# Fytex/Shafa-CD

Measured on AMD Instinct MI355X. Metric: GiB/s Shannon-Fano encode+decode, 64 MiB blocks, 1/2/4/8 GPUs; bit-exact, higher is better.
Workload: dtype u8

## Files before the change

### shafa-cd_amd/csrc/sf_decode.hip

```cpp
#include <type_traits>
#include "common.hpp"
#include "internal.hpp"

#include <atomic>
#include <mutex>
#include <thread>

#include <algorithm>

#include <stdlib.h>

#include "sfd_common.hpp"
#include "sfd_dp.hpp"
#include "sfd_generic.hpp"

namespace {

typedef __attribute__((address_space(3))) u32 lds_u32;
typedef __attribute__((address_space(3))) u16 lds_u16;
typedef __attribute__((address_space(3))) u8 lds_u8;
template <int LONG> constexpr u32 spec_emask() { return LONG == 2 ? 31u : 15u; }

constexpr int SC_PHW = 16;
constexpr int SC_M = 4;
// ... 470 lines not shown
{
    const u32 mask = (1u << KW) - 1u;
    auto long_len = [&](const u32 qq) -> u32 {
        const u32 win = __builtin_bitreverse32(sw.at(qq));
        const u32 l = (LONG == 1 ? long_code(lt, win) : long_code32(lt, win)) >> 8;
        return l ? l : 1u;
    };
    const u32 nlook = KW <= 10 ? 3u : 2u;
    while (q + nlook * KW <= qe && (int)(q + nlook * KW) <= qlimit) {
        const u32 w = sw.at(q);
        u32 sum = 0, e = 0;
        for (u32 i = 0; i < nlook; ++i) {
            e = tab[(w >> (sum & 31u)) & mask];
            sum += e;
        }
        q += sum & 31u;
        cnt += sum >> 5;
        if (LONG && __builtin_expect((e & 31u) == 0u, 0)) {
            const u32 l = long_len(q);
            if ((int)(q + l) > qlimit) { q = qe + spec_emask<LONG>(); return; }
            q += l;
            ++cnt;
        }
    }
    const lds_u8 *len0 = tab + (1u << KW);
    while (q < qe) {
        u32 l0 = len0[sw.at(q) & mask];
        if (LONG && __builtin_expect(l0 == 0u, 0)) l0 = long_len(q);
        if ((int)(q + l0) > qlimit) { q = qe + spec_emask<LONG>(); break; }
        q += l0;
        ++cnt;
    }
}

template <bool HAVE_OLD, int LONG>
__device__ __forceinline__ void sl_strip(const lds_u8 *tab, const u16 *lt, const u32 KW, const u32 qrow, const int qlimit, const u32 ent0,
                                         u32 (&ent)[2], u32 (&cnt)[2], u32 &exit_)
{
    u32 q = qrow + ent0;
    SlWin sw;
    sw.init();
#pragma unroll
    for (int k = 0; k < 2; ++k) {
        const u32 r = q - (qrow + 256u * k);
        if (HAVE_OLD && k > 0 && r == ent[k]) return;
        ent[k] = r;
        u32 c = 0;
        sl_walk<LONG>(tab, lt, KW, q, qrow + 256u * (k + 1), qlimit, c, sw);
        cnt[k] = c;
    }
    exit_ = (q - (qrow + 512u)) & spec_emask<LONG>();
}

template <int LONG>
__device__ __forceinline__ u32 sl_region(u8 *smem, const DecBlk &blk, const u32 tile0, const u32 e0_forced, u8 *__restrict__ chunk_entry,
                                         u16 *__restrict__ chunk_cnt, u32 *__restrict__ tile_cnt, u8 *__restrict__ tile_guess,
                                         u8 *__restrict__ tile_exit, const u32 tab_bytes)
{
    const u64 start = (u64)tile0 * DTILE;
    const u64 left = blk.in_n > start ? blk.in_n - start : 0;
    const size_t gt0 = (size_t)blk.tile_base + tile0;
    const u32 ntl = blk.n_tiles - tile0 < (u32)SC_WTILES ? blk.n_tiles - tile0 : (u32)SC_WTILES;
    u32 *data = (u32 *)smem;
    const u32 tab_off = SL_LDS_DATA;
    u8 *ex = smem + SL_LDS_DATA + tab_bytes;
    const u32 tid = threadIdx.x, lane = tid & 63, wv = tid >> 6;
    const u32 KW = blk.KW;
    const u16 *lt = (const u16 *)(smem + SL_LDS_DATA + tab_bytes + SL_MISC);
    {
        const long long base = (long long)start - 4 * SL_SW;
        constexpr u32 UNITS = (u32)(SL_STRIPS * SL_SW / 4 + 1), NIT = (UNITS + DEC_THREADS - 1) / DEC_THREADS;
        uint4 v[NIT];
#pragma unroll
        for (u32 it = 0; it < NIT; ++it) {
            const u32 i = tid + it * DEC_THREADS;
            const long long off = base + (long long)i * 16;
            v[it] = make_uint4(0, 0, 0, 0);
            if (i < UNITS && off >= 0 && (u64)off + 16 <= blk.in_n) v[it] = gload<uint4>(blk.in + off);
        }
#pragma unroll
        for (u32 it = 0; it < NIT; ++it) {
            const u32 i = tid + it * DEC_THREADS;
            if (i >= UNITS) break;
            const long long off = base + (long long)i * 16;
            u32 w[4] = {v[it].x, v[it].y, v[it].z, v[it].w};
            if (off >= 0 && (u64)off < blk.in_n && (u64)off + 16 > blk.in_n) {
                const int nv = (int)(blk.in_n - (u64)off);
#pragma unroll
                for (int q = 0; q < 16; ++q)
                    if (q < nv) w[q >> 2] |= (u32)gload<u8>(blk.in + off + q) << (8 * (q & 3));
            }
            const u32 f = 4 * i, at = f + f / SL_SW;
            const u32 w0 = rev_bytes(w[0]);
            if (f % SL_SW == 0 && f > 0) data[at - 1] = w0;
            if (i < UNITS - 1) {
                data[at] = w0;
                data[at + 1] = rev_bytes(w[1]);
                data[at + 2] = rev_bytes(w[2]);
                data[at + 3] = rev_bytes(w[3]);
            }
        }
    }
    __syncthreads();
    const int limit = (int)(left * 8) - (int)(512u * tid);
    const u32 qrow = 8u * ((4u * SL_ROW) * (tid + 1));
    const int qlimit = (int)qrow + limit;
    const lds_u8 *tab = (const lds_u8 *)(size_t)tab_off;
    u32 ent[2] = {0, 0}, cnt[2] = {0, 0}, exit_ = 0;
    {
        u32 e0;
        if (tid == 0) e0 = e0_forced;
        else {
            const u32 qe = qrow;
            u32 q = qe - 256u, dummy = 0;
            SlWin sw;
            sw.init();
            sl_walk<LONG>(tab, lt, KW, q, qe, qlimit, dummy, sw);
            e0 = (q - qe) & spec_emask<LONG>();
        }
        sl_strip<false, LONG>(tab, lt, KW, qrow, qlimit, e0, ent, cnt, exit_);
    }
    ex[tid] = (u8)exit_;
    __syncthreads();
    bool bad = false;
    u32 *const wsum = (u32 *)(ex + DEC_THREADS), *const flags = wsum + 4;
    u32 turn = 0;
    for (int round = 0; round < 4; ++round) {
        bad = tid > 0 && ent[0] != (u32)ex[tid - 1];
        if (!wg_any(bad, flags, turn)) break;
        if (bad) sl_strip<true, LONG>(tab, lt, KW, qrow, qlimit, (u32)ex[tid - 1], ent, cnt, exit_);
        __syncthreads();
        ex[tid] = (u8)exit_;
        __syncthreads();
        bad = tid > 0 && ent[0] != (u32)ex[tid - 1];
    }
    if (wg_any(bad, flags, turn)) {
        if (tid == 0) __hip_atomic_store(blk.run_dp, 1u, __ATOMIC_RELAXED, __HIP_MEMORY_SCOPE_AGENT);
    }
    const u32 my_tile = tid / 128u;
    const u32 wtot = dpp_scan_add(cnt[0] + cnt[1]);
    if (lane == 63) wsum[wv] = wtot;
    __syncthreads();
    if (my_tile < ntl) {
        const size_t c0 = gt0 * DEC_THREADS + (size_t)tid * 2;
        gstore<u16>(chunk_entry + c0, (u16)((ent[0] & 0xFFu) | (ent[1] << 8)));
        gstore<u32>(chunk_cnt + c0, cnt[0] | (cnt[1] << 16));
        const u32 in_tile = tid & 127u;
        if (in_tile == 0) {
            tile_cnt[gt0 + my_tile] = wsum[2 * my_tile] + wsum[2 * my_tile + 1];
            tile_guess[gt0 + my_tile] = (u8)ent[0];
        }
        if (in_tile == 127u) tile_exit[gt0 + my_tile] = (u8)exit_;
    }
    const u32 unit_exit = ex[ntl * 128u - 1u];
    __syncthreads();
    return unit_exit;
}

constexpr u32 SF_CHUNKS = 8;

constexpr u32 SF_LINKS = 2 * DEC_THREADS;
template <int LONG>
__device__ __forceinline__ void sf_links(u8 *smem, const DecBlk &blk, const u32 t_begin, const u32 t_end, u8 *__restrict__ chunk_entry,
                                         u16 *__restrict__ chunk_cnt, u32 *__restrict__ tile_cnt, u8 *__restrict__ tile_guess,
                                         const u8 *__restrict__ tile_exit, const u32 tab_bytes, const u32 long_bytes)
{
    const u32 tid = threadIdx.x, KW = blk.KW, mask = (1u << KW) - 1u;
    const u16 *lt = (const u16 *)(smem + tab_bytes + 48);
    const u8 *len0 = smem + (1u << KW);
    const u64 end_bit = blk.in_n * 8;
    u32 turn = 0;
    u32 xs[SF_LINKS / DEC_THREADS];
    bool any_bad = false;
#pragma unroll
    for (u32 i = 0; i < SF_LINKS / DEC_THREADS; ++i) {
        const u32 t = t_begin + tid + i * DEC_THREADS;
        xs[i] = 0xFFFFFFFFu;
        if (t < t_end) {
            const size_t gt = (size_t)blk.tile_base + t;
            const u32 x = tile_exit[gt - 1];
            if (tile_guess[gt] != x) { xs[i] = x; any_bad = true; }
        }
    }
    if (!wg_any(any_bad, (u32 *)(smem + tab_bytes), turn)) return;
    __syncthreads();
    fill_lds16((void *)smem, (const void *)blk.cnt3, 2u << KW);
    if (LONG) {
        const u16 *src = LONG == 1 ? blk.longtab : blk.long32;
        if (src) fill_lds16((void *)lt, src, long_bytes);
        else if (tid == 0) *(u16 *)lt = 0;
    }
    bool failed = false;
    volatile u32 *const gave_up = (volatile u32 *)(smem + tab_bytes + 32);
    if (tid == 0) *gave_up = 0;
    __syncthreads();
#pragma unroll 1
    for (u32 i = 0; i < SF_LINKS / DEC_THREADS; ++i) {
        if (*gave_up) break;
        const u32 x = xs[i];
        if (x == 0xFFFFFFFFu) continue;
        const u32 t = t_begin + tid + i * DEC_THREADS;
        const size_t gt = (size_t)blk.tile_base + t;
        const u64 tile_bit0 = (u64)t * DTILE * 8;
        if (x >= spec_emask<LONG>() || tile_bit0 + (u64)(SF_CHUNKS + 1) * CH_BITS + 64 > end_bit) { failed = true; *gave_up = 1; continue; }
        u32 q = x, wi = 0xFFFFFFFFu, lo = 0, hi = 0;
        auto window = [&](const u32 qq) -> u32 {
            const u32 i = qq >> 5;
            if (i != wi) {
                const u8 *p = blk.in + (u64)t * DTILE + 4u * i;
                lo = rev_bytes(gload<u32>(p));
                hi = rev_bytes(gload<u32>(p + 4));
                wi = i;
            }
            return __builtin_amdgcn_alignbit(hi, lo, qq);
        };
        int delta = 0;
        bool merged = false;
        const size_t c0 = gt * DEC_THREADS;
        for (u32 c = 0; c < SF_CHUNKS; ++c) {
            const u32 qe = CH_BITS * (c + 1);
            u32 cnt = 0;
            while (q < qe) {
                const u32 w = window(q);
                u32 l = len0[w & mask];
                if (LONG && l == 0u) {
                    const u32 win = __builtin_bitreverse32(w);
                    l = (LONG == 1 ? long_code(lt, win) : long_code32(lt, win)) >> 8;
                    if (!l) l = 1u;
                }
                q += l;
                ++cnt;
            }
            delta += (int)cnt - (int)chunk_cnt[c0 + c];
            chunk_cnt[c0 + c] = (u16)cnt;
            const u32 e = q - qe;
            if (e == (u32)chunk_entry[c0 + c + 1]) { merged = true; break; }
            chunk_entry[c0 + c + 1] = (u8)e;
        }
        if (!merged) { failed = true; *gave_up = 1; continue; }
        chunk_entry[c0] = (u8)x;
        tile_guess[gt] = (u8)x;
        tile_cnt[gt] = (u32)((int)tile_cnt[gt] + delta);
    }
    if (wg_any(failed, (u32 *)(smem + tab_bytes), turn) && tid == 0)
        __hip_atomic_store(blk.run_dp, 1u, __ATOMIC_RELAXED, __HIP_MEMORY_SCOPE_AGENT);
}

template <int LONG>
__global__ __launch_bounds__(DEC_THREADS) void sfd_ends(const DecBlk *__restrict__ blks, u8 *__restrict__ chunk_entry,
                                                        u16 *__restrict__ chunk_cnt, u32 *__restrict__ tile_cnt,
                                                        u8 *__restrict__ tile_guess, u8 *__restrict__ tile_exit, u32 tab_bytes, u32 long_bytes)
{
    extern __shared__ __attribute__((aligned(16))) u8 smem[];
    const DecBlk blk = blks[blockIdx.y];
    if (!blk.n_tiles || !blk.run_dp || __hip_atomic_load(blk.run_dp, __ATOMIC_RELAXED, __HIP_MEMORY_SCOPE_AGENT) != 0) return;
    if (lds_addr(smem) != 0) __builtin_trap();
    const u32 units = (blk.n_tiles + SC_WTILES - 1) / SC_WTILES;
    u32 first_end = units - 1;
    if (units >= 2 && blk.in_n - (u64)(units - 2) * SC_WTILES * DTILE < (u64)64 * SC_SB + 4) first_end = units - 2;
    if (blockIdx.x > 0) {
        const u32 t_end = first_end * SC_WTILES, t_begin = 1u + (blockIdx.x - 1u) * SF_LINKS;
        if (t_begin < t_end)
            sf_links<LONG>(smem, blk, t_begin, t_end, chunk_entry, chunk_cnt, tile_cnt, tile_guess, tile_exit, tab_bytes, long_bytes);
        return;
    }
    fill_lds16((void *)(smem + SL_LDS_DATA), (const void *)blk.cnt3, 2u << blk.KW);
    if (LONG) {
        u16 *lt = (u16 *)(smem + SL_LDS_DATA + tab_bytes + SL_MISC);
        const u16 *src = LONG == 1 ? blk.longtab : blk.long32;
        if (src) fill_lds16((void *)lt, src, long_bytes);
        else if (threadIdx.x == 0) *lt = 0;
    }
    __syncthreads();
    u32 e0 = first_end ? (u32)tile_exit[(size_t)blk.tile_base + first_end * SC_WTILES - 1] : 0u;
    for (u32 u = first_end; u < units; ++u)
        e0 = sl_region<LONG>(smem, blk, u * SC_WTILES, e0, chunk_entry, chunk_cnt, tile_cnt, tile_guess, tile_exit, tab_bytes);
}

constexpr int ws_row(bool esc) { return CH_BYTES / 4 + (esc ? 3 : 2); }
constexpr int ws_rows_bytes(bool esc)
{
    return 16 + (DEC_THREADS * ws_row(esc) + (esc ? 0 : DEC_THREADS / 16)) * 4;
}
constexpr int WS_MISC = 32;
typedef unsigned int u32x3_t __attribute__((ext_vector_type(3)));
constexpr u32 WS_NST = 4, WS_DROP = 0x7FFFFFF0u;
constexpr int WS_RSRC_FLAGS = 0x00020000, WS_AUX_NT = 2;

__device__ __forceinline__ void ws_walk1(const u32 tab_off, const u32 mask2, const u32 xa, u32 q2, const u32 q2end, u32 want,
                                         const bool by_pos)
{
    auto window2 = [&]() -> u32 {
        const lds_u32 *pa = (const lds_u32 *)(size_t)((q2 >> 3) & ~3u);
        return __builtin_amdgcn_alignbit(pa[1], pa[0], q2);
    };
    auto look = [&](const u32 w) -> u32 { return *(const lds_u16 *)(size_t)(tab_off + (w & mask2)); };
    auto image_or = [](const u32 at, const u32 v) {
        __hip_atomic_fetch_or((lds_u32 *)(size_t)at, v, __ATOMIC_RELAXED, __HIP_MEMORY_SCOPE_WORKGROUP);
    };
    if (by_pos) {
        constexpr u32 N = 3, F = 4, WPG = F * N / 4;
        const u32 s = (0u - xa) & 3u;
        u32 ptr = ((xa + 3u) & ~3u) - 4u;
        u32 L = 0, Lp = 0, Ep = 0;
        auto group = [&](auto first_group) -> bool {
            constexpr bool FIRST = decltype(first_group)::value;
            u32 x0 = 0, x1 = 0, ub = 0;
#pragma unroll
            for (u32 f = 0; f < F; ++f) {
                if (!((int)q2 < (int)q2end)) {
                    if (f == 0) {
                        if (!FIRST) {
                            image_or(ptr + 4u * (WPG - 1u), Ep);
                            image_or(ptr + 4u * WPG, __builtin_amdgcn_alignbyte(0u, Lp, s));
                        }
                    } else {
                        const u32 at = ptr + 4u * (f * N >> 2);
                        image_or(at, __builtin_amdgcn_alignbyte(L, Lp, s));
                        image_or(at + 4u, __builtin_amdgcn_alignbyte(0u, L, s));
                    }
                    return false;
                }
                if (f == 0 && !FIRST) {
                    *(lds_u32 *)(size_t)(ptr + 4u * (WPG - 1u)) = Ep;
                    ptr += 4u * WPG;
                }
                u32 w;
                if ((f & 1u) == 0) {
                    const lds_u32 *pa = (const lds_u32 *)(size_t)((q2 >> 3) & ~3u);
                    const u32 w0 = pa[0], w1 = pa[1], w2 = pa[2];
                    w = x0 = __builtin_amdgcn_alignbit(w1, w0, q2);
                    x1 = __builtin_amdgcn_alignbit(w2, w1, q2);
                } else
                    w = __builtin_amdgcn_alignbit(x1, x0, ub);
                u32 ua = 0;
#pragma unroll
                for (u32 i = 0; i < N; ++i) {
                    const u32 k = f * N + i, b = k & 3u;
                    const u32 e = look(w >> ua);
                    ua += e >> 8;
                    L = __builtin_amdgcn_perm(e, L, b == 0 ? 0x0C0C0C04u : b == 1 ? 0x0C0C0400u : b == 2 ? 0x0C040100u : 0x04020100u);
                    if (b == 3u) {
                        const u32 E = __builtin_amdgcn_alignbyte(L, Lp, s), at = ptr + 4u * (k >> 2);
                        Lp = L;
                        if (FIRST && k == 3u) image_or(at, E);
                        else if (k == F * N - 1u) Ep = E;
                        else *(lds_u32 *)(size_t)at = E;
                    }
                }
                q2 += ua;
                ub = ua;
            }
            return true;
        };
        if (group(std::true_type{}))
            while (group(std::false_type{})) {}
        return;
    }
    u32 wp = xa & ~3u, nb = 8u * (xa & 3u), acc = 0;
    for (; want; --want) {
        const u32 e = look(window2());
        q2 += e >> 8;
        acc |= (e & 0xFFu) << nb;
        nb += 8u;
        if (nb == 32u) {
            image_or(wp, acc);
            wp += 4u;
            acc = nb = 0;
        }
    }
    if (nb) image_or(wp, acc);
}

template <int LONG, bool ESC, bool ONE = false>
__global__ __launch_bounds__(DEC_THREADS) void sfd_wstage(const DecBlk *__restrict__ blks, const u8 *__restrict__ chunk_entry,
                                                          const u16 *__restrict__ chunk_cnt, const u64 *__restrict__ tile_off,
                                                          u32 tpw, u32 tab_bytes, u32 cap, u32 long_bytes)
{
    extern __shared__ __attribute__((aligned(16))) u8 smem[];
    const DecBlk blk = blks[blockIdx.y];
    const u32 first_tile = blockIdx.x * tpw;
    if (first_tile >= blk.n_tiles) return;
    if (tile_off[(size_t)blk.tile_base + first_tile] >= blk.n_sym) return;
    const u32 LONGB = LONG ? long_bytes : 0u;
    u32 *rows = (u32 *)(smem + 16);
    constexpr u32 WS_ROW = (u32)ws_row(ESC), tab_off = (u32)ws_rows_bytes(ESC);
    const u16 *lt = (const u16 *)(smem + tab_off + tab_bytes);
    const u32 img_off = tab_off + tab_bytes + LONGB;
    u32 *wsum = (u32 *)(smem + img_off + cap);
    u32 *next = wsum + 4;
    const u32 tid = threadIdx.x, lane = tid & 63, wv = tid >> 6;
    const u32 K1 = blk.K1, K3 = sym3_window(K1);
    const u32 sh = 32 - K1;
    static_assert(!ONE || (LONG == 0 && !ESC), "the one-code walk has no escapes");
    constexpr bool one = ONE;
    fill_lds16(smem + tab_off, (const void *)blk.sym3, (one ? 2u : 4u) << K3);
    if (LONG) {
        const u16 *src = LONG == 1 ? blk.longtab : blk.long32;
        if (src) fill_lds16((void *)lt, src, LONGB);
        else if (tid == 0) *(u16 *)lt = 0;
    }
    for (u32 i = tid; i < cap / 16; i += DEC_THREADS) *(uint4 *)(smem + img_off + 16 * i) = make_uint4(0, 0, 0, 0);
    bool bad = false;
    if (lds_addr(smem) != 0) __builtin_trap();
    const u32 q2row = 8u * (16u + 4u * (WS_ROW * tid + (ESC ? 0u : tid >> 4))) - (one ? 1u : 2u);
    const u32 mask4 = ((1u << K3) - 1u) << (one ? 1 : 2);
    auto fetch16 = [&](const u64 off) -> uint4 {
        if (off + 16 <= blk.in_n) return gload_nt<uint4>(blk.in + off);
        u32 w[4] = {0, 0, 0, 0};
        if (off < blk.in_n) {
            const int nv = (int)(blk.in_n - off);
#pragma unroll
            for (int q = 0; q < 16; ++q)
                if (q < nv) w[q >> 2] |= (u32)gload<u8>(blk.in + off + q) << (8 * (q & 3));
        }
        return make_uint4(w[0], w[1], w[2], w[3]);
    };
    uint4 pf0, pf1;
    u32 pf2[ESC ? 3 : 2] = {};
    auto fetch_ahead = [&](const u64 off) {
        constexpr int NB = ESC ? 12 : 8;
        if (off + NB <= blk.in_n) {
            if constexpr (ESC) {
                const u32x3_t v = __builtin_nontemporal_load((const GLOBAL_AS u32x3_t *)(unsigned long long)(blk.in + off));
                pf2[0] = v.x; pf2[1] = v.y; pf2[2] = v.z;
            } else {
                const uint2 v = gload_nt<uint2>(blk.in + off);
                pf2[0] = v.x; pf2[1] = v.y;
            }
            return;
        }
        u32 w[3] = {0, 0, 0};
        if (off < blk.in_n) {
            const int nv = (int)(blk.in_n - off);
#pragma unroll
            for (int q = 0; q < NB; ++q)
                if (q < nv) w[q >> 2] |= (u32)gload<u8>(blk.in + off + q) << (8 * (q & 3));
        }
#pragma unroll
        for (int q = 0; q < NB / 4; ++q) pf2[q] = w[q];
    };
    u8 pf_entry = 0, pf_next = 0;
    u16 pf_cnt = 0;
    auto prefetch = [&](const u32 tile) {
        const u64 base = (u64)tile * DTILE;
        const size_t g = ((size_t)blk.tile_base + tile) * DEC_THREADS + tid;
        pf_entry = chunk_entry[g];
        pf_cnt = chunk_cnt[g];
        pf_next = (tile + 1 < blk.n_tiles || tid + 1 < (u32)DEC_THREADS) ? chunk_entry[g + 1] : (u8)0;
        pf0 = fetch16(base + 16ull * tid);
        pf1 = fetch16(base + 16ull * (tid + DEC_THREADS));
        if (tid == 0) fetch_ahead(base + DTILE);
    };
    auto put16 = [&](const u32 i, const uint4 v) {
        const u32 f = 4 * i, at = f + (WS_ROW - 8u) * (f >> 3) + (ESC ? 0u : f >> 7);
        const u32 w0 = rev_bytes(v.x), w1 = rev_bytes(v.y), w2 = rev_bytes(v.z);
        if ((f & 7u) == 0 && f > 0) {
            const u32 lk = at - (WS_ROW - 8u) - (!ESC && (f & 127u) == 0 ? 1u : 0u);
            rows[lk] = w0;
            rows[lk + 1] = w1;
            if (ESC) rows[lk + 2] = w2;
        }
        if (i < (u32)(DTILE / 16)) {
            rows[at] = w0;
            rows[at + 1] = w1;
            rows[at + 2] = w2;
            rows[at + 3] = rev_bytes(v.w);
        }
    };
    auto store_bytes = [&](u8 *ga, const uint4 v, const u32 lo, const u32 hi) {
        const u32 wds[4] = {v.x, v.y, v.z, v.w};
#pragma unroll
        for (u32 q = 0; q < 16; ++q)
            if (q >= lo && q < hi) gstore<u8>(ga + q, (u8)(wds[q >> 2] >> (8 * (q & 3))));
    };
    u32 carry_n = 0, carry_lo = 0;
    u8 *carry_g = nullptr;
    prefetch(first_tile);
    __builtin_amdgcn_s_waitcnt(0x0F70);
    for (u32 it = 0; it < tpw; ++it) {
        const u32 tile = first_tile + it;
        if (tile >= blk.n_tiles) break;
        const size_t gt = (size_t)blk.tile_base + tile;
        const u64 toff = tile_off[gt];
        if (toff >= blk.n_sym) break;
        lds_barrier();
        put16(tid, pf0);
        put16(tid + DEC_THREADS, pf1);
        if (tid == 0) put16(DTILE / 16, make_uint4(pf2[0], pf2[1], ESC ? pf2[ESC ? 2 : 0] : 0u, 0u));
        const u32 entry = pf_entry, cnt = pf_cnt, nent = pf_next;
        if (it + 1 < tpw && tile + 1 < blk.n_tiles) prefetch(tile + 1);
        const u32 incl = wave_incl_scan_add<u32>(cnt);
        if (lane == 63) wsum[wv] = incl;
        lds_barrier();
        u32 pre = incl - cnt, total = 0;
        for (u32 w = 0; w < 4; ++w) { if (w < wv) pre += wsum[w]; total += wsum[w]; }
        const u64 room = blk.n_sym - toff;
        const u32 tot_c = (u32)__builtin_amdgcn_readfirstlane((int)(room < (u64)total ? (u32)room : total));
        u32 want = pre >= tot_c ? 0u : (tot_c - pre < cnt ? tot_c - pre : cnt);
        u32 q2 = q2row + entry;
        const bool by_pos = want == cnt && tile + 1 < blk.n_tiles && nent != spec_emask<LONG>();
        const u32 q2end = q2row + 256u + nent;
        u32 done = 0;
        do {
            u8 *gout = blk.out + toff + done;
            const u32 mis = (u32)((uintptr_t)gout & 15u);
            if (carry_g && (carry_n != mis || carry_g != gout - mis)) {
                if (tid == 0) {
                    uint4 *ip = (uint4 *)(smem + img_off);
                    store_bytes(carry_g, *ip, carry_lo, carry_n);
                    ip[0] = make_uint4(0, 0, 0, 0);
                    ip[1] = make_uint4(0, 0, 0, 0);
                }
                carry_n = 0;
                carry_g = nullptr;
                lds_barrier();
            }
            const u32 capw = cap - 32;
            u32 nxt = tot_c;
            if (mis + (tot_c - done) > capw) {
                if (tid == 0) *next = tot_c;
                lds_barrier();
                if (want && pre >= done && mis + (pre - done) + want > capw) atomicMin(next, pre);
                lds_barrier();
                nxt = (u32)__builtin_amdgcn_readfirstlane((int)*next);
                lds_barrier();
            }
            const bool mine = want && pre >= done && pre + want <= nxt;
            if constexpr (ONE) {
                if (mine) ws_walk1(tab_off, mask4, img_off + mis + (pre - done), q2, q2end, want, by_pos);
            } else if (mine) {
                const u32 x = mis + (pre - done);
                u32 wp = img_off + (x & ~3u), nbx = x << 30, acc = 0;
                auto emit = [&](const u32 e) {
                    const u32 sh = nbx >> 27, syms = e & 0xFFFFFFu;
                    acc |= syms << sh;
                    if (__builtin_add_overflow(nbx, e & 0xC0000000u, &nbx)) {
                        __hip_atomic_fetch_or((lds_u32 *)(size_t)wp, acc, __ATOMIC_RELAXED, __HIP_MEMORY_SCOPE_WORKGROUP);
                        wp += 4u;
                        acc = syms >> (32u - sh);
                    }
                };
                auto window4 = [&]() -> u32 {
                    const lds_u32 *pa = (const lds_u32 *)(size_t)((q2 >> 3) & ~3u);
                    return __builtin_amdgcn_alignbit(pa[1], pa[0], q2);
                };
                auto step = [&](const bool tail) {
                    u32 e = *(const lds_u32 *)(size_t)(tab_off + (window4() & mask4));
                    if (ESC && __builtin_expect((e >> 30) == 0, 0)) {
                        const u32 q = q2 + 2u;
                        const lds_u32 *pb = (const lds_u32 *)(size_t)((q >> 3) & ~3u);
                        const u32 win = __builtin_bitreverse32(__builtin_amdgcn_alignbit(pb[1], pb[0], q));
                        u32 e1 = LONG == 1 ? long_code(lt, win) : LONG == 2 ? long_code32(lt, win)
                                           : (u32)gload<u16>(blk.lut13 + (win >> sh));
                        if (e1 == 0) { bad = true; e1 = 1u << 8; }
                        e = (e1 & 0xFFu) | ((e1 >> 8) << 24) | (1u << 30);
                    }
                    u32 n = e >> 30, syms = e & 0xFFFFFFu;
                    if (tail) {
                        n = n < want ? n : want;
                        syms &= (1u << (8 * n)) - 1u;
                    }
                    emit(syms | n << 30);
                    q2 += (e >> 24) & 63u;
                    want -= n;
                };
                auto multi = [&](auto nlook) {
                    constexpr u32 N = decltype(nlook)::value;
                    if (by_pos) {
                        while ((int)q2 < (int)q2end) {
                            const u32 w4 = window4();
                            u32 ua = 0, e = 0;
#pragma unroll
                            for (u32 i = 0; i < N; ++i) {
                                e = *(const lds_u32 *)(size_t)(tab_off + ((w4 >> (ua & 31u)) & mask4));
                                emit(e);
                                ua += e >> 24;
                            }
                            q2 += ua & 63u;
                            if (ESC && __builtin_expect((e >> 30) == 0, 0)) step(false);
                        }
                        want = 0;
                    }
                    while (want >= 3 * N) {
                        const u32 w4 = window4();
                        u32 ua = 0, e = 0;
#pragma unroll
                        for (u32 i = 0; i < N; ++i) {
                            e = *(const lds_u32 *)(size_t)(tab_off + ((w4 >> (ua & 31u)) & mask4));
                            emit(e);
                            ua += e >> 24;
                        }
                        q2 += ua & 63u;
                        want -= ua >> 6;
                        if (ESC && __builtin_expect((e >> 30) == 0, 0)) step(false);
                    }
                };
                if (K3 <= 10) multi(std::integral_constant<u32, 3>{});
                else if (K3 <= 15) multi(std::integral_constant<u32, 2>{});
                while (want) step(true);
                if (nbx) __hip_atomic_fetch_or((lds_u32 *)(size_t)wp, acc, __ATOMIC_RELAXED, __HIP_MEMORY_SCOPE_WORKGROUP);
            }
            lds_barrier();
            const u32 end = mis + (nxt - done);
            const u32 lo0 = (carry_n == mis && carry_n) ? carry_lo : mis;
            const u32 nfull = end >> 4;
            u8 *const g0 = gout - mis;
            if constexpr (LONG == 2) {
                for (u32 u = tid; u < nfull; u += DEC_THREADS) {
                    uint4 *ip = (uint4 *)(smem + img_off + 16 * u);
                    const uint4 v = *ip;
                    *ip = make_uint4(0, 0, 0, 0);
                    if (u == 0 && lo0) store_bytes(g0, v, lo0, 16u);
                    else gstore_nt<uint4>(g0 + 16 * u, v);
                }
            } else {
                const __amdgpu_buffer_rsrc_t win = __builtin_amdgcn_make_buffer_rsrc(g0, 0, (int)(16u * nfull), WS_RSRC_FLAGS);
                u32 ub = tid;
                do {
#pragma unroll
                    for (u32 s = 0; s < WS_NST; ++s) {
                        const u32 u = ub + s * DEC_THREADS;
                        u32x4_t x = {0u, 0u, 0u, 0u};
                        u32 off = WS_DROP;
                        if (u < nfull) {
                            uint4 *ip = (uint4 *)(smem + img_off + 16 * u);
                            const uint4 v = *ip;
                            *ip = make_uint4(0, 0, 0, 0);
                            if (s == 0 && u == 0 && lo0) store_bytes(g0, v, lo0, 16u);
                            else {
                                x.x = v.x; x.y = v.y; x.z = v.z; x.w = v.w;
                                off = 16u * u;
                            }
                        }
                        __builtin_amdgcn_raw_buffer_store_b128(x, win, (int)off, 0, WS_AUX_NT);
                    }
                    ub += WS_NST * DEC_THREADS;
                } while (__builtin_amdgcn_readfirstlane((int)(ub - tid)) < (int)nfull);
            }
            if (tid == 0 && nfull) {
                uint4 *ip = (uint4 *)(smem + img_off);
                const uint4 a = ip[nfull], b = ip[nfull + 1];
                ip[nfull] = make_uint4(0, 0, 0, 0);
                ip[nfull + 1] = make_uint4(0, 0, 0, 0);
                ip[0] = a;
                ip[1] = b;
            }
            carry_lo = nfull ? 0u : lo0;
            carry_n = end & 15u;
            carry_g = g0 + 16 * nfull;
            done = nxt;
            if (done < tot_c) lds_barrier();
        } while (done < tot_c);
    }
    if (tid == 0 && carry_n) {
        const uint4 v = *(const uint4 *)(smem + img_off);
        store_bytes(carry_g, v, carry_lo, carry_n);
    }
    if (bad) set_error(blk.err, SHAFA_FILE_UNRECOGNIZABLE);
}

__global__ __launch_bounds__(DEC_THREADS) void sfd_offsets(const DecBlk *__restrict__ blks,
                                                           const u32 *__restrict__ tile_cnt, u64 *__restrict__ tile_off)
{
    __shared__ u64 wtot[4];
    __shared__ u64 carry;
    const DecBlk blk = blks[blockIdx.x];
    const u32 tid = threadIdx.x, lane = tid & 63, wv = tid >> 6;
    if (tid == 0) carry = 0;
    __syncthreads();
    constexpr u32 OFF_EPT = 16;
    for (u32 r0 = 0; r0 < blk.n_tiles; r0 += DEC_THREADS * OFF_EPT) {
        const u32 t0 = r0 + tid * OFF_EPT;
        u32 x[OFF_EPT];
#pragma unroll
        for (u32 j = 0; j < OFF_EPT; ++j) x[j] = t0 + j < blk.n_tiles ? tile_cnt[blk.tile_base + t0 + j] : 0u;
        u64 mine = 0;
#pragma unroll
        for (u32 j = 0; j < OFF_EPT; ++j) mine += x[j];
        const u64 incl = wave_incl_scan_add<u64>(mine);
        if (lane == 63) wtot[wv] = incl;
        __syncthreads();
        u64 base = carry + incl - mine;
        for (u32 w = 0; w < wv; ++w) base += wtot[w];
#pragma unroll
        for (u32 j = 0; j < OFF_EPT; ++j) {
            if (t0 + j < blk.n_tiles) tile_off[blk.tile_base + t0 + j] = base;
            base += x[j];
        }
        __syncthreads();
        if (tid == 0) carry += wtot[0] + wtot[1] + wtot[2] + wtot[3];
        __syncthreads();
    }
    if (tid == 0 && carry < blk.n_sym) set_error(blk.err, SHAFA_FILE_UNRECOGNIZABLE);
}

}

#include "sfd_host_tables.hpp"

template <class F> static void for_blocks_parallel(int nblocks, F fn)
{
    std::atomic<int> next{0};
    auto work = [&]() {
        for (;;) {
            const int b = next.fetch_add(1, std::memory_order_relaxed);
            if (b >= nblocks) break;
            fn(b);
        }
    };
    int helpers = nblocks / 16;
    const int hw = (int)std::thread::hardware_concurrency();
    if (helpers > 7) helpers = 7;
    if (hw > 0 && helpers > hw - 1) helpers = hw - 1;
    std::vector<std::thread> th;
    for (int i = 0; i < helpers; ++i) {
        try { th.emplace_back(work); } catch (...) { break; }
    }
    work();
    for (auto &t : th) t.join();
}

static int g_sfd_speculate = 1;
void sfdec_configure(int speculate) { g_sfd_speculate = speculate; }
static int g_sfd_path = 0;
void sfdec_configure_path(int path) { g_sfd_path = path; }

static bool spec_worthwhile(const shafa_code_table &t, const HostTab &h, bool force)
{
    if (!h.ok || !(h.complete || h.complete16 || h.complete32) || h.lmax > 32 || h.lmax < 2) return false;
    if (force) return true;
    const u64 key = spec_key(t.len, t.bits);
    static u64 ckey[1024];
    static signed char cval[1024];
    static std::mutex cmu;
    const u32 slot = (u32)(key >> 17) & 1023u;
    {
        std::lock_guard<std::mutex> lk(cmu);
        if (cval[slot] && ckey[slot] == key) return cval[slot] == 2;
    }
    u64 rs = key | 1ull;
    int fails = 0;
    for (int trial = 0; trial < SPEC_TRIALS && fails <= SPEC_MAX_FAILS; ++trial) {
        u64 w[SPEC_WORDS];
        for (u64 &x : w) x = spec_rand(rs);
        if (!spec_trial(w, h.lenlut.data(), h.K1)) ++fails;
    }
    const bool yes = fails <= SPEC_MAX_FAILS;
    std::lock_guard<std::mutex> lk(cmu);
    ckey[slot] = key;
    cval[slot] = yes ? 2 : 1;
    return yes;
}

struct SfdArrays {
    u8 *cfn, *tfn;
    u8 *tent, *cent;
    u16 *ccnt;
    u32 *tcnt;
    u64 *toff;
    u8 *tguess, *texit;
};

enum SfdForm { SFD_MID32, SFD_LONG_ALL, SFD_PACKED12, SFD_PACKED13, SFD_PACKED };

static u32 sfd_tpw(u32 most, u32 max_tiles, int nblocks)
{
    u32 tpw = most;
    while (tpw > 1 && (u64)ceil_div_u64(max_tiles, tpw) * nblocks < 2048) tpw >>= 1;
    return tpw;
}

static void sfd_launch_packed(hipStream_t st, const DecBlk *dblk, int nblocks, u32 max_tiles, SfdForm form, bool esc, bool spec,
                              u32 tabb, u32 long_used, bool all_spec, u32 ws_tab, u32 ws_cap, const SfdArrays &a, bool one = false)
{
    static decltype(&sfd_scan<0>) const scans[3] = {sfd_scan<2>, sfd_scan<1>, sfd_scan<0>};
    static decltype(&sfd_ends<0>) const ends[3] = {sfd_ends<2>, sfd_ends<1>, sfd_ends<0>};
    static decltype(&sfd_sync16<true, false>) const syncs[4] = {sfd_sync16<false, true>, sfd_sync16<true, false, 12>,
                                                                sfd_sync16<true, false, 13>, sfd_sync16<true, false>};
    const int f = form < SFD_PACKED12 ? form : 2;
    const dim3 grid_b((u32)nblocks), wg(DEC_THREADS);
    hipLaunchKernelGGL(sfd_tables, dim3((u32)nblocks, 8), wg, 0, st, dblk);
    if (spec) {
        const size_t lds_scan = (size_t)SC_LDS_ROWS + tabb + SC_MISC + long_used;
        const size_t lds_ends = (size_t)SL_LDS_DATA + tabb + SL_MISC + long_used;
        hipLaunchKernelGGL(scans[f], dim3((u32)ceil_div_u64(max_tiles, SC_TILES), (u32)nblocks), wg, lds_scan, st, dblk, a.cent, a.ccnt,
                           a.tcnt, a.tguess, a.texit, tabb, long_used);
        hipLaunchKernelGGL(ends[f], dim3(1u + (u32)ceil_div_u64(max_tiles, SF_LINKS), (u32)nblocks), wg, lds_ends, st, dblk, a.cent,
                           a.ccnt, a.tcnt, a.tguess, a.texit, tabb, long_used);
    }
    const u32 tpw = all_spec ? 256u : sfd_tpw(4, max_tiles, nblocks);
    const dim3 grid_f((u32)ceil_div_u64(max_tiles, tpw), (u32)nblocks);
    if (form == SFD_MID32) {
        hipLaunchKernelGGL(sfd_sync32, grid_f, wg, 0, st, dblk, a.cfn, a.tfn, tpw);
        hipLaunchKernelGGL(sfd_tiles, grid_b, wg, (size_t)32 * DEC_THREADS + DEC_THREADS, st, dblk, 32u, (const u8 *)a.tfn, a.tent);
        hipLaunchKernelGGL(sfd_countfsm32, grid_f, wg, 0, st, dblk, (const u8 *)a.cfn, (const u8 *)a.tent, a.cent, a.ccnt, a.tcnt, tpw);
    } else {
        constexpr int CSUBS = 4;
        hipLaunchKernelGGL(syncs[form - SFD_LONG_ALL], grid_f, wg, 0, st, dblk, (u64 *)a.cfn, (u64 *)a.tfn, tpw);
        hipLaunchKernelGGL(sfd_tiles16, grid_b, wg, 0, st, dblk, (const u64 *)a.tfn, a.tent);
        hipLaunchKernelGGL((sfd_countfsm<CSUBS>), dim3((u32)ceil_div_u64(max_tiles, tpw * CSUBS), (u32)nblocks), dim3(DEC_THREADS * CSUBS),
                           0, st, dblk, (const u64 *)a.cfn, (const u8 *)a.tent, a.cent, a.ccnt, a.tcnt, tpw);
    }
    hipLaunchKernelGGL(sfd_offsets, grid_b, wg, 0, st, dblk, (const u32 *)a.tcnt, a.toff);
    static decltype(&sfd_wstage<0, false>) const wstages[5] = {sfd_wstage<2, true>, sfd_wstage<1, true>, sfd_wstage<0, true>,
                                                               sfd_wstage<0, false>, sfd_wstage<0, false, true>};
    const u32 tpw_ws = sfd_tpw(16, max_tiles, nblocks);
    const size_t lds_ws = (size_t)ws_rows_bytes(esc) + ws_tab + ws_cap + WS_MISC + long_used;
    hipLaunchKernelGGL(wstages[one ? 4 : f == 2 && !esc ? 3 : f], dim3((u32)ceil_div_u64(max_tiles, tpw_ws), (u32)nblocks), wg, lds_ws, st,
                       dblk, (const u8 *)a.cent, (const u16 *)a.ccnt, (const u64 *)a.toff, tpw_ws, ws_tab, ws_cap, long_used);
}

static int sfd_launch_bytemap(hipStream_t st, const DecBlk *dblk, u32 nb, u32 max_tiles, u32 R, u32 l2cap, const SfdArrays &a)
{
    const size_t lds_lut = (size_t)(1u << LUT_MAXK) * 2 + (size_t)l2cap * 2;
    const size_t lds_sync = (size_t)LDS_DATA + (size_t)R * DEC_THREADS + lds_lut + 4 * R + 64;
    const size_t lds_count = lds_sync + DEC_THREADS;
    const size_t lds_write = (size_t)LDS_DATA + lds_lut + 64;
    const size_t lds_tiles = (size_t)R * DEC_THREADS + DEC_THREADS;
    if (lds_tiles > 65536 || lds_sync > 65536) {
        HIP_TRY(hipFuncSetAttribute((const void *)sfd_sync, hipFuncAttributeMaxDynamicSharedMemorySize, (int)lds_sync));
        HIP_TRY(hipFuncSetAttribute((const void *)sfd_count, hipFuncAttributeMaxDynamicSharedMemorySize, (int)lds_count));
        HIP_TRY(hipFuncSetAttribute((const void *)sfd_tiles, hipFuncAttributeMaxDynamicSharedMemorySize, (int)lds_tiles));
    }
    const dim3 grid_t(max_tiles, nb), grid_b(nb), wg(DEC_THREADS);
    hipLaunchKernelGGL(sfd_sync, grid_t, wg, lds_sync, st, dblk, R, l2cap, a.cfn, a.tfn);
    hipLaunchKernelGGL(sfd_tiles, grid_b, wg, lds_tiles, st, dblk, R, (const u8 *)a.tfn, a.tent);
    hipLaunchKernelGGL(sfd_count, grid_t, wg, lds_count, st, dblk, R, l2cap, (const u8 *)a.cfn, (const u8 *)a.tent, a.cent, a.ccnt,
                       a.tcnt);
    hipLaunchKernelGGL(sfd_offsets, grid_b, wg, 0, st, dblk, (const u32 *)a.tcnt, a.toff);
    hipLaunchKernelGGL(sfd_write, grid_t, wg, lds_write, st, dblk, l2cap, (const u8 *)a.cent, (const u16 *)a.ccnt, (const u64 *)a.toff);
    return SHAFA_SUCCESS;
}

int sfdec_launch(Batch *bt, hipStream_t st, int nblocks, const u8 *d_in, const u64 *h_in_off,
                 const u64 *h_in_n, const shafa_code_table *h_tables, const u64 *h_n_symbols, u8 *d_out,
                 const u64 *h_out_off)
{
    if (nblocks <= 0) return SHAFA_SUCCESS;
    if (nblocks > bt->max_blocks) return SHAFA_LACK_OF_MEMORY;

    std::vector<HostTab> tabs(nblocks);
    u32 lmax_all = 1, max_tiles = 0, max_l2 = 0;
    u64 total_tiles = 0;
    size_t tab_bytes = 0;
    std::vector<u32> ntiles(nblocks, 0);
    bool pair_all = true;
    bool c16_all = true;
    bool c32_all = true;
    for (int b = 0; b < nblocks; ++b)
        if ((h_in_off[b] & 15) || (h_out_off[b] & 15)) return SHAFA_OUTSIDE_MODULE;
    {
        std::atomic<bool> nomem{false};
        for_blocks_parallel(nblocks, [&](int b) {
            try { build_host_tab(h_tables[b], tabs[b]); } catch (...) { nomem.store(true); }
        });
        if (nomem.load()) return SHAFA_LACK_OF_MEMORY;
    }
    for (int b = 0; b < nblocks; ++b) {
        HostTab &h = tabs[b];
        bool run = h_n_symbols[b] > 0;
        if (run && (!h.ok || h.empty)) {
            bt->h_hosterr[b] = SHAFA_FILE_UNRECOGNIZABLE;
            run = false;
        }
        if (run && h_in_n[b] == 0) { bt->h_hosterr[b] = SHAFA_FILE_UNRECOGNIZABLE; run = false; }
        if (!run) continue;
        ntiles[b] = (u32)ceil_div_u64(h_in_n[b], DTILE);
        total_tiles += ntiles[b];
        if (ntiles[b] > max_tiles) max_tiles = ntiles[b];
        if (h.lmax > lmax_all) lmax_all = h.lmax;
        tab_bytes += ((h.lut.size() * 2 + 15) & ~(size_t)15) + ((h.trie.size() * 4 + 15) & ~(size_t)15) +
                     ((h.lenlut.size() + 15) & ~(size_t)15) + ((h.lut2.size() * 2 + 16 + 15) & ~(size_t)15) +
                     ((h.lut13.size() * 2 + 15) & ~(size_t)15) + (h.longtab.empty() ? 0 : (size_t)LONG_BYTES) +
                     (h.long32.empty() ? 0 : (size_t)((LONG32_BYTES + 15) & ~15)) + ((h.lenlut32.size() + 15) & ~(size_t)15);
        if (h.lut2.size() > max_l2) max_l2 = (u32)h.lut2.size();
        pair_all = pair_all && h.complete;
        c16_all = c16_all && h.complete16;
        c32_all = c32_all && (h.complete16 || h.complete32);
    }
    if (!total_tiles) return SHAFA_SUCCESS;
    u32 R = 16;
    while (R < lmax_all) R <<= 1;
    if (g_sfd_path >= 1) pair_all = c16_all = c32_all = false;
    const bool long_all = R == 16 && !pair_all && c16_all && lmax_all > (u32)LEN_MAXK;
    const bool packed = R == 16 && ((pair_all && lmax_all <= (u32)LEN_MAXK) || long_all);
    const bool mid32 = !packed && R == 32 && c32_all;
    const bool ws_esc = mid32 || long_all || lmax_all > (u32)SYM3_MAXK;
    bool ws_one = !ws_esc;
    for (int b = 0; b < nblocks; ++b)
        if (ntiles[b] && !tabs[b].one) ws_one = false;
    if (!packed && !mid32 && R < 32) R = 32;

    size_t off = 0;
    const size_t o_blk = off; off += ((size_t)nblocks * sizeof(DecBlk) + 15) & ~(size_t)15;
    const size_t o_rundp = off; off += ((size_t)nblocks * 4 + 15) & ~(size_t)15;
    const size_t o_tab = off; off += tab_bytes;
    const size_t stage_bytes = off;
    const size_t o_tilefn = off; off += (size_t)total_tiles * (R < 8 ? 8 : R); off = (off + 15) & ~(size_t)15;
    const size_t o_tent = off; off += (size_t)total_tiles; off = (off + 15) & ~(size_t)15;
    const size_t o_tcnt = off; off += (size_t)total_tiles * 4; off = (off + 15) & ~(size_t)15;
    const size_t o_toff = off; off += (size_t)total_tiles * 8;
    const size_t o_cent = off; off += (size_t)total_tiles * DEC_THREADS; off = (off + 15) & ~(size_t)15;
    const size_t o_ccnt = off; off += (size_t)total_tiles * DEC_THREADS * 2; off = (off + 15) & ~(size_t)15;
    const bool need_tabs = packed || mid32;
    const size_t o_pair = off; off += (packed && pair_all) ? (size_t)nblocks * (2u << LEN_MAXK) : 0;
    const size_t o_cnt3 = off; off += need_tabs ? (size_t)nblocks * (2u << LEN_MAXK) : 0;
    const size_t o_sym3 = off; off += need_tabs ? (size_t)nblocks * (4u << LEN_MAXK) : 0;
    const size_t o_fsm4 = off; off += need_tabs ? (size_t)nblocks * 16384 : 0;
    const size_t o_fsm1 = off; off += need_tabs ? (size_t)nblocks * 2048 : 0;
    const size_t o_cfn = off; off += packed ? (size_t)total_tiles * DEC_THREADS * 8 : (size_t)total_tiles * R * DEC_THREADS;
    const bool spec_path = (packed || mid32) && g_sfd_speculate != 0;
    std::vector<u32> hblk_kw(nblocks, 0);
    for (int b = 0; b < nblocks; ++b) {
        if (!ntiles[b]) continue;
        u32 n13 = 0;
        if (tabs[b].K1 == 13)
            for (int sy = 0; sy < 256; ++sy) n13 += h_tables[b].len[sy] == 13;
        hblk_kw[b] = scan_window(tabs[b].K1, long_all || mid32, n13);
    }
    u32 long_used = 0;
    if (long_all) {
        u32 gmax = 0;
        for (int b = 0; b < nblocks; ++b)
            if (ntiles[b] && !tabs[b].longtab.empty() && tabs[b].longtab[0] > gmax) gmax = tabs[b].longtab[0];
        long_used = (16u + (u32)LONG_PFX * 2u + gmax * 32u + 15u) & ~15u;
    } else if (mid32) {
        u32 nmax = 0;
        for (int b = 0; b < nblocks; ++b)
            if (ntiles[b] && !tabs[b].long32.empty() && tabs[b].long32[1] > nmax) nmax = tabs[b].long32[1];
        long_used = (16u + (u32)LONG_PFX * 4u + nmax * 4u + 15u) & ~15u;
    }
    std::vector<char> spec_blk(nblocks, 0);
    bool any_spec = false;
    for (int b = 0; spec_path && b < nblocks; ++b)
        if (ntiles[b] && spec_worthwhile(h_tables[b], tabs[b], g_sfd_speculate == 2)) { spec_blk[b] = 1; any_spec = true; }
    const size_t o_tguess = off; off += any_spec ? (size_t)total_tiles : 0; off = (off + 15) & ~(size_t)15;
    const size_t o_texit = off; off += any_spec ? (size_t)total_tiles : 0; off = (off + 15) & ~(size_t)15;
    int rc = batch_reserve(bt, st, off);
    if (rc) return rc;
    u8 *ws = (u8 *)bt->d_ws;

    u8 *dpar = batch_params_begin(bt, stage_bytes);
    if (!dpar) return SHAFA_LACK_OF_MEMORY;
    ParamsScope pscope(bt, st);
    u8 *hs = (u8 *)batch_stage(bt, bt->par_inline ? st : bt->copy_st, stage_bytes);
    if (!hs) return SHAFA_LACK_OF_MEMORY;
    DecBlk *hb = (DecBlk *)hs;
    size_t tpos = o_tab;
// ... 125 lines not shown
```

Measured before the change: 894.7.

## Replace LDS atomic-OR image assembly with plain stores in single-walker decode path

In the ONE decode path, the by-position walker now writes boundary words with ordinary stores and byte/halfword stores instead of LDS atomic ORs. The output image no longer has to be zeroed after every flush. A block-wide ballot decides whether the whole tile can take the store-only path. When it cannot, the image is explicitly cleared (keeping the carried prefix bytes) before walking. This is meant to cut LDS atomic and zeroing traffic, at the cost of an extra clearing pass and a barrier on partial tiles.

Result: no change. 903.5, median of 6 (+1.0%).

```diff
diff --git a/shafa-cd_amd/csrc/sf_decode.hip b/shafa-cd_amd/csrc/sf_decode.hip
--- a/shafa-cd_amd/csrc/sf_decode.hip
+++ b/shafa-cd_amd/csrc/sf_decode.hip
@@ -796,27 +796,25 @@
         constexpr u32 N = 3, F = 4, WPG = F * N / 4;
         const u32 s = (0u - xa) & 3u;
         u32 ptr = ((xa + 3u) & ~3u) - 4u;
-        u32 L = 0, Lp = 0, Ep = 0;
+        u32 L = 0, Lp = 0;
+        u32 fo = 0;
+        auto put_bytes = [](const u32 a, const u32 v, const u32 nn, const bool half_first) {
+            const u32 one_at = half_first ? (nn & 2u) : 0u, half_at = half_first ? 0u : (nn & 1u);
+            if (nn & 1u) *(lds_u8 *)(size_t)(a + one_at) = (u8)(v >> (8u * one_at));
+            if (nn & 2u) *(lds_u16 *)(size_t)(a + half_at) = (u16)(v >> (8u * half_at));
+        };
         auto group = [&](auto first_group) -> bool {
             constexpr bool FIRST = decltype(first_group)::value;
             u32 x0 = 0, x1 = 0, ub = 0;
 #pragma unroll
             for (u32 f = 0; f < F; ++f) {
-                if (!((int)q2 < (int)q2end)) {
-                    if (f == 0) {
-                        if (!FIRST) {
-                            image_or(ptr + 4u * (WPG - 1u), Ep);
-                            image_or(ptr + 4u * WPG, __builtin_amdgcn_alignbyte(0u, Lp, s));
-                        }
-                    } else {
-                        const u32 at = ptr + 4u * (f * N >> 2);
-                        image_or(at, __builtin_amdgcn_alignbyte(L, Lp, s));
-                        image_or(at + 4u, __builtin_amdgcn_alignbyte(0u, L, s));
-                    }
+                if (!FIRST && !((int)q2 < (int)q2end)) {
+                    fo = 4u * (f == 0 ? WPG - 1u : f * N >> 2);
                     return false;
                 }
                 if (f == 0 && !FIRST) {
-                    *(lds_u32 *)(size_t)(ptr + 4u * (WPG - 1u)) = Ep;
+                    *(lds_u32 *)(size_t)(ptr + 4u * (WPG - 1u)) = __builtin_amdgcn_alignbyte(L, Lp, s);
+                    Lp = L;
                     ptr += 4u * WPG;
                 }
                 u32 w;
@@ -834,12 +832,10 @@
                     const u32 e = look(w >> ua);
                     ua += e >> 8;
                     L = __builtin_amdgcn_perm(e, L, b == 0 ? 0x0C0C0C04u : b == 1 ? 0x0C0C0400u : b == 2 ? 0x0C040100u : 0x04020100u);
-                    if (b == 3u) {
-                        const u32 E = __builtin_amdgcn_alignbyte(L, Lp, s), at = ptr + 4u * (k >> 2);
+                    if (b == 3u && k != F * N - 1u) {
+                        if (FIRST && k == 3u) put_bytes(xa, L, s, false);
+                        else *(lds_u32 *)(size_t)(ptr + 4u * (k >> 2)) = __builtin_amdgcn_alignbyte(L, Lp, s);
                         Lp = L;
-                        if (FIRST && k == 3u) image_or(at, E);
-                        else if (k == F * N - 1u) Ep = E;
-                        else *(lds_u32 *)(size_t)at = E;
                     }
                 }
                 q2 += ua;
@@ -847,8 +843,16 @@
             }
             return true;
         };
-        if (group(std::true_type{}))
-            while (group(std::false_type{})) {}
+        group(std::true_type{});
+        while (group(std::false_type{})) {}
+        const u32 at = ptr + fo;
+        const u32 A = __builtin_amdgcn_alignbyte(L, Lp, s), Bw = __builtin_amdgcn_alignbyte(0u, L, s);
+        const u32 xe = xa + want, B = xe & ~3u;
+        if (B != at) {
+            *(lds_u32 *)(size_t)at = A;
+            if (B != at + 4u) *(lds_u32 *)(size_t)(at + 4u) = Bw;
+        }
+        put_bytes(B, B == at ? A : Bw, xe, true);
         return;
     }
     u32 wp = xa & ~3u, nb = 8u * (xa & 3u), acc = 0;
@@ -986,6 +990,10 @@
         if (it + 1 < tpw && tile + 1 < blk.n_tiles) prefetch(tile + 1);
         const u32 incl = wave_incl_scan_add<u32>(cnt);
         if (lane == 63) wsum[wv] = incl;
+        if constexpr (ONE) {
+            const bool part = __builtin_amdgcn_ballot_w64(cnt < 12u || nent == spec_emask<LONG>()) != 0;
+            if (lane == 63) ((u8 *)(wsum + 5))[wv] = part ? 1 : 0;
+        }
         lds_barrier();
         u32 pre = incl - cnt, total = 0;
         for (u32 w = 0; w < 4; ++w) { if (w < wv) pre += wsum[w]; total += wsum[w]; }
@@ -993,7 +1001,12 @@
         const u32 tot_c = (u32)__builtin_amdgcn_readfirstlane((int)(room < (u64)total ? (u32)room : total));
         u32 want = pre >= tot_c ? 0u : (tot_c - pre < cnt ? tot_c - pre : cnt);
         u32 q2 = q2row + entry;
-        const bool by_pos = want == cnt && tile + 1 < blk.n_tiles && nent != spec_emask<LONG>();
+        bool by_pos;
+        if constexpr (ONE)
+            by_pos = tile + 1 < blk.n_tiles && __builtin_amdgcn_readfirstlane((int)wsum[5]) == 0 &&
+                     tot_c == (u32)__builtin_amdgcn_readfirstlane((int)total);
+        else
+            by_pos = want == cnt && tile + 1 < blk.n_tiles && nent != spec_emask<LONG>();
         const u32 q2end = q2row + 256u + nent;
         u32 done = 0;
         do {
@@ -1019,6 +1032,20 @@
                 lds_barrier();
                 nxt = (u32)__builtin_amdgcn_readfirstlane((int)*next);
                 lds_barrier();
+            }
+            if constexpr (ONE) {
+                if (!by_pos) {
+                    for (u32 i = tid + 1; i < cap / 16; i += DEC_THREADS) *(uint4 *)(smem + img_off + 16 * i) = make_uint4(0, 0, 0, 0);
+                    if (tid == 0) {
+                        u32 *p0 = (u32 *)(smem + img_off);
+#pragma unroll
+                        for (int w = 0; w < 4; ++w) {
+                            const int keep = (int)mis - 4 * w;
+                            if (keep < 4) p0[w] = keep <= 0 ? 0u : p0[w] & ((1u << (8 * keep)) - 1u);
+                        }
+                    }
+                    lds_barrier();
+                }
             }
             const bool mine = want && pre >= done && pre + want <= nxt;
             if constexpr (ONE) {
@@ -1120,7 +1147,7 @@
                         if (u < nfull) {
                             uint4 *ip = (uint4 *)(smem + img_off + 16 * u);
                             const uint4 v = *ip;
-                            *ip = make_uint4(0, 0, 0, 0);
+                            if constexpr (!ONE) *ip = make_uint4(0, 0, 0, 0);
                             if (s == 0 && u == 0 && lo0) store_bytes(g0, v, lo0, 16u);
                             else {
                                 x.x = v.x; x.y = v.y; x.z = v.z; x.w = v.w;
@@ -1134,11 +1161,14 @@
             }
             if (tid == 0 && nfull) {
                 uint4 *ip = (uint4 *)(smem + img_off);
-                const uint4 a = ip[nfull], b = ip[nfull + 1];
-                ip[nfull] = make_uint4(0, 0, 0, 0);
-                ip[nfull + 1] = make_uint4(0, 0, 0, 0);
-                ip[0] = a;
-                ip[1] = b;
+                if constexpr (ONE) ip[0] = ip[nfull];
+                else {
+                    const uint4 a = ip[nfull], b = ip[nfull + 1];
+                    ip[nfull] = make_uint4(0, 0, 0, 0);
+                    ip[nfull + 1] = make_uint4(0, 0, 0, 0);
+                    ip[0] = a;
+                    ip[1] = b;
+                }
             }
             carry_lo = nfull ? 0u : lo0;
             carry_n = end & 15u;
```
